# MarioPasc/MGA-YOLO

Measured on AMD Instinct MI355X. Metric: images/s (MaskCBAM fwd+bwd step at P3/P4/P5, YOLOv8n 640x640), higher is better.
Workload: dtype f32

## Files before the change

mga_yolo_amd/csrc/api_bwd.hip:

```cpp
#include "host.cuh"
#include "bwd.cuh"

static int backward_args(const mgacbam_bwd_level_t& L, BwdArgs& A, Sig& sig) {
  if (!L.x || !L.gy || !L.ctx || !L.scratch || !L.gx) return fail(MGACBAM_E_NULL, "backward: x / gy / ctx / scratch / gx is NULL");
  if (!L.gw1 || !L.gb1 || !L.gw2 || !L.gb2 || !L.gwsa || !L.gbeta) return fail(MGACBAM_E_NULL, "backward: NULL parameter-gradient pointer");
  if (L.gmask && !L.mask) return fail(MGACBAM_E_NULL, "backward: gmask requested but mask is NULL");
  if (int e = check_params(L.p)) return e;
  if (int e = check_shape(L.B, L.C, L.H, L.W, L.p.hidden, L.p.k)) return e;
  if (L.dtype < MGACBAM_F32 || L.dtype > MGACBAM_BF16) return fail(MGACBAM_E_DTYPE, "backward: dtype %d", L.dtype);
  const int VEC = vec_of(L.H, L.W, L.dtype);
  const size_t need = VEC * elem_size(L.dtype);
  if (!aligned_to(L.x, need) || !aligned_to(L.gy, need) || !aligned_to(L.gx, need) || !aligned_to(L.ctx, 16) ||
      !aligned_to(L.scratch, 16) || (L.gmask && !aligned_to(L.gmask, 16)))
    return fail(MGACBAM_E_ALIGN, "backward: x/gy/gx must be %zu-byte aligned, ctx/scratch 16-byte", need);
  A.x = L.x; A.mask = L.mask; A.gy = L.gy; A.gx = L.gx; A.gmask = L.gmask;
  A.gw1 = L.gw1; A.gb1 = L.gb1; A.gw2 = L.gw2; A.gb2 = L.gb2; A.gwsa = L.gwsa; A.gbeta = L.gbeta;
  A.c = ctx_ptrs(const_cast<void*>(L.ctx), L.B, L.C, L.H, L.W, L.p.hidden);
  A.p = make_params(L.p);
  A.g = make_geo(L.B, L.C, L.H, L.W, L.p);
  A.t = choose_tune(L.B, L.C, L.H, L.W, L.p.k, L.dtype);
  const ScratchLayout SL = scratch_layout(L.B, L.C, L.H, L.W, L.p.hidden, L.p.k, L.dtype);
  {
    mgacbam_ctx_layout_t CL;
    ctx_layout(L.B, L.C, L.H, L.W, L.p.hidden, &CL);
    if (int e = check_capacity("backward", "ctx", static_cast<size_t>(CL.total), L.ctx_bytes)) return e;
    if (int e = check_capacity("backward", "scratch", SL.total, L.scratch_bytes)) return e;
  }
  char* sp = static_cast<char*>(L.scratch);
  A.s.A_part = reinterpret_cast<float*>(sp + SL.A_part);
  A.s.gpre = reinterpret_cast<float*>(sp + SL.gpre); A.s.gplanes = reinterpret_cast<float*>(sp + SL.gplanes);
  A.s.gwsa_part = reinterpret_cast<float*>(sp + SL.gwsa_part);
  A.s.gz = reinterpret_cast<float*>(sp + SL.gz); A.s.gbq = reinterpret_cast<float*>(sp + SL.gbq);
  A.s.gh_avg = reinterpret_cast<float*>(sp + SL.gh_avg); A.s.gh_mx = reinterpret_cast<float*>(sp + SL.gh_mx);
  A.s.pgh = reinterpret_cast<float*>(sp + SL.pgh);
  A.nt = chan_tiles(A.t, A.g.H, A.g.W, VEC);
  A.nconv = A.g.B * conv_tiles(A.t, A.g.H, A.g.W);
  A.nwsa = A.g.B * wsa_tiles(A.t, A.g.H, A.g.W);
  A.nrole = A.nwsa;
  A.wsa_tail = 0;
  A.npg = params_blocks(A.g);
  A.ncg = 0;
  A.nflag = static_cast<int>(sync_flags(static_cast<size_t>(L.H) * L.W));
  A.bflag0 = L.B * A.nflag + 4 + L.B;
  A.cflag0 = A.bflag0 + L.B * A.nflag;
  A.mbflag0 = A.cflag0 + L.B * A.nflag; A.mcflag0 = A.mbflag0 + L.B * A.nflag;
  A.wflag0 = A.mcflag0 + L.B * A.nflag; A.sflag0 = A.wflag0 + L.B * A.nflag;
  A.merged = 0;
  A.vec = VEC;
  { const Knobs kn = knobs(); A.trace = kn.trace; A.spin_limit = kn.spin_limit; }
  const int proj = (L.flags & MGACBAM_BWD_HAVE_PROJ) && L.gmask != nullptr;
  A.g.proj_h = (proj && L.p.hidden <= MGACBAM_PROJ_MAX_HIDDEN) ? L.p.hidden : 0;
  sig = Sig{L.dtype, VEC, L.mask != nullptr, L.p.k, L.gmask != nullptr, proj};
  return 0;
}

static int backward_group(BwdArgs* lv, int n, const Sig& sig, int stages, hipStream_t st) {
  Group<BwdArgs> G;
  G.n = n;
  const int r2max = knobs().r2_cpt == 1 || knobs().r2_cpt == 2 || knobs().r2_cpt == 4 ? knobs().r2_cpt : 4;
  const int cpt = group_cpt(lv, n, r2max);
  for (int l = 0; l < n; ++l) {
    lv[l].t.pool_cpt = cpt;
    const int cpb = (kBlock / lv[l].t.pool_tx) * cpt;
    lv[l].ncg = (lv[l].g.C + cpb - 1) / cpb;
    G.lv[l] = lv[l];
  }
  auto fill = [&](auto blocks_of) { int tot = 0; for (int l = 0; l < n; ++l) { G.start[l] = tot; tot += blocks_of(lv[l]); } G.start[n] = tot; return tot; };

  bool fold = (stages & MGACBAM_BWD_FOLD) && (stages & MGACBAM_BWD_REDUCE1) && (stages & MGACBAM_BWD_CONVT) && knobs().bwd_fold;
  for (int l = 0; l < n && fold; ++l) {
    const int TP = lv[l].t.chan_tx * sig.vec;
    fold = TP >= kSyncPx && TP >= lv[l].g.W && 8 * (((lv[l].t.conv_th + lv[l].g.k) * lv[l].g.W + TP - 1) / TP + 1) <= 512 &&
           lv[l].nconv <= lv[l].g.B * lv[l].nflag;
  }
  const bool fuse_early = (stages & MGACBAM_BWD_FUSE) != 0;
  const bool tail_early = fuse_early && (stages & MGACBAM_BWD_APPLY) && (stages & MGACBAM_BWD_PARAMGRAD) && (stages & MGACBAM_BWD_WSA) && sig.k == 7 &&
                          knobs().wsa_tail;
  bool merge = fold && fuse_early && (stages & MGACBAM_BWD_REDUCE2) && (stages & MGACBAM_BWD_WSA) && sig.k == 7 && !tail_early && knobs().bwd_merge &&
               !knobs().wsa_fat;
  for (int l = 0; l < n && merge; ++l) merge = lv[l].nwsa <= lv[l].g.B * lv[l].nflag && lv[l].ncg <= lv[l].g.C && lv[l].nconv % lv[l].g.B == 0;
  if (merge) {
    R12Group R;
    R.g.n = n;
    size_t smem = 0;
    for (int l = 0; l < n; ++l) {
      lv[l].merged = 1; lv[l].bflag0 = lv[l].mbflag0; lv[l].cflag0 = lv[l].mcflag0; lv[l].nrole = lv[l].nwsa;
      R.g.lv[l] = lv[l];
      smem = std::max({smem, reduce1_smem(lv[l].g, sig.vec), convT_smem(lv[l].t, sig.k), wsa_smem(lv[l].t, sig.k),
                       (64 + static_cast<size_t>(std::max(kPghLds, kBlock / lv[l].t.pool_tx))) * sizeof(float)});
    }
    int tot = 0;
    for (int p = 0; p < 4; ++p) {
      for (int l = 0; l < n; ++l) {
        R.seg[p][l] = tot;
        tot += p == 0 ? xcd_grid(lv[l].g.B, lv[l].nt) : p == 1 ? pad8(lv[l].nconv) : p == 2 ? pad8(lv[l].nwsa) : sweep_blocks(lv[l], lv[l].t.pool_tx, cpt);
      }
      R.seg[p][n] = tot;
    }
    const int grid = tot;
#define CALL_R12B(CPTV) LAUNCH((k_bwd_r12<TT, VV, CPTV>), grid, smem, st, R)
#define CALL_R12(Tt, Vv) { using TT = Tt; constexpr int VV = Vv; DISPATCH_CPT(cpt, CALL_R12B); }
    DISPATCH_T_VEC(sig.dtype, sig.vec, CALL_R12);
#undef CALL_R12
#undef CALL_R12B
    if (int e = launch_status("k_bwd_r12")) return e;
    for (int l = 0; l < n; ++l) G.lv[l] = lv[l];
  }
  if (fold && !merge) {
    size_t smem = 0;
    for (int l = 0; l < n; ++l) smem = std::max({smem, reduce1_smem(lv[l].g, sig.vec), convT_smem(lv[l].t, sig.k)});
    const int grid = fill([&](const BwdArgs& a) { return xcd_grid(a.g.B, a.nt) + pad8(a.nconv); });
#define CALL_R1F(Tt, Vv) if (sig.k == 7) LAUNCH((k_bwd_reduce1_fold<Tt, Vv, 7>), grid, smem, st, G); else LAUNCH((k_bwd_reduce1_fold<Tt, Vv, 0>), grid, smem, st, G)
    DISPATCH_T_VEC(sig.dtype, sig.vec, CALL_R1F);
#undef CALL_R1F
    if (int e = launch_status("k_bwd_reduce1_fold")) return e;
  }
  if ((stages & MGACBAM_BWD_REDUCE1) && !fold) {
    size_t smem = 0;
    for (int l = 0; l < n; ++l) smem = std::max(smem, reduce1_smem(lv[l].g, sig.vec));
    const int grid = fill([&](const BwdArgs& a) { return xcd_grid(a.g.B, a.nt); });
#define CALL_R1(Tt, Vv) LAUNCH((k_bwd_reduce1<Tt, Vv>), grid, smem, st, G)
    DISPATCH_T_VEC(sig.dtype, sig.vec, CALL_R1);
#undef CALL_R1
    if (int e = launch_status("k_bwd_reduce1")) return e;
  }
  if ((stages & MGACBAM_BWD_CONVT) && !fold) {
    size_t smem = 0;
    for (int l = 0; l < n; ++l) smem = std::max(smem, convT_smem(lv[l].t, sig.k));
    const int grid = fill([&](const BwdArgs& a) { return a.nconv; });
    switch (sig.k) {
      case 3: LAUNCH(k_bwd_convT<3>, grid, smem, st, G); break;
      case 5: LAUNCH(k_bwd_convT<5>, grid, smem, st, G); break;
      case 7: LAUNCH(k_bwd_convT<7>, grid, smem, st, G); break;
      default: LAUNCH(k_bwd_convT<0>, grid, smem, st, G); break;
    }
    if (int e = launch_status("k_bwd_convT")) return e;
  }
  const bool fuse = (stages & MGACBAM_BWD_FUSE) != 0;
  const bool fuse_pg = fuse && (stages & MGACBAM_BWD_APPLY) && (stages & MGACBAM_BWD_PARAMGRAD);
  const bool wsa_tail = fuse_pg && (stages & MGACBAM_BWD_FOLD) && (stages & MGACBAM_BWD_WSA) && sig.k == 7 && knobs().wsa_tail;
  const bool fuse_wsa = fuse && (stages & MGACBAM_BWD_REDUCE2) && (stages & MGACBAM_BWD_WSA) && sig.k == 7 && !wsa_tail;
  if (wsa_tail) for (int l = 0; l < n; ++l) { lv[l].wsa_tail = 1; G.lv[l].wsa_tail = 1; }
  if ((stages & MGACBAM_BWD_REDUCE2) && !merge) {
    size_t smem = 0;
    for (int l = 0; l < n; ++l) {
      smem = std::max(smem, (64 + static_cast<size_t>(std::max(kPghLds, kBlock / lv[l].t.pool_tx))) * sizeof(float));
      if (fuse_wsa) smem = std::max(smem, wsa_smem(lv[l].t, sig.k));
    }
    if (fuse_wsa && knobs().wsa_fat) {
      int slots = 0;
#define RES_R22(CPTV) slots = resident_workgroups(k_bwd_reduce2<TT, VV, CPTV, true>, smem)
#define RES_R2(Tt, Vv) { using TT = Tt; constexpr int VV = Vv; DISPATCH_CPT(cpt, RES_R22); }
      DISPATCH_T_VEC(sig.dtype, sig.vec, RES_R2);
#undef RES_R2
#undef RES_R22
      long long streaming = 0, tiles = 0;
      for (int l = 0; l < n; ++l) {
        const int cpb = (kBlock / lv[l].t.pool_tx) * cpt;
        streaming += static_cast<long long>(lv[l].g.B) * ((lv[l].g.C + cpb - 1) / cpb);
        tiles += lv[l].nwsa;
      }
      const long long idle = slots - streaming;
      if (idle >= 32 && idle < tiles) {
        for (int l = 0; l < n; ++l) {
          lv[l].nrole = static_cast<int>(std::max(1ll, std::min<long long>(lv[l].nwsa, idle * lv[l].nwsa / tiles)));
          G.lv[l].nrole = lv[l].nrole;
        }
      }
    }
    const int grid = fill([&](const BwdArgs& a) { return (fuse_wsa ? pad8(a.nrole) : 0) + sweep_blocks(a, a.t.pool_tx, cpt); });
#define CALL_R22(CPTV) if (fuse_wsa) LAUNCH((k_bwd_reduce2<TT, VV, CPTV, true>), grid, smem, st, G); else LAUNCH((k_bwd_reduce2<TT, VV, CPTV, false>), grid, smem, st, G)
#define CALL_R2(Tt, Vv) { using TT = Tt; constexpr int VV = Vv; DISPATCH_CPT(cpt, CALL_R22); }
    DISPATCH_T_VEC(sig.dtype, sig.vec, CALL_R2);
#undef CALL_R2
#undef CALL_R22
    if (int e = launch_status("k_bwd_reduce2")) return e;
  }
  if ((stages & MGACBAM_BWD_WSA) && !fuse_wsa && !wsa_tail && !merge) {
    size_t smem = 0;
// ... 52 lines not shown
```

mga_yolo_amd/csrc/args.cuh:

```cuda
#pragma once
#include <stddef.h>
#include <stdint.h>

namespace mgacbam {

struct Geo {
  int B, C, H, W, HW;
  int hidden, k;
  int use_sigmoid;
  float thr, eps;
  int proj_h;
};
constexpr int kProjMax = 4;
#ifndef MGACBAM_GATE_R
#define MGACBAM_GATE_R 16
#endif
constexpr int kGateR = MGACBAM_GATE_R;
constexpr int kSyncPx = 16;

struct CtxPtrs {
  float* S; float* use; float* den;
  float* avg; float* mx; float* mavg;
  int* valid; int* amax;
  float* h_avg; float* h_mx; float* ca;
// ... 9 lines not shown
  int pool_cpt;
  int chan_tx;
  int chanf_tx;
  int conv_twq;
  int conv_th;
  int wsa_th;
  int apply_rows;
  int nt_stores;
  int gate_rows;
  int gate_tx;
  int gate_span;
};

struct FwdArgs {
  const void* x; const float* mask; void* y;
  CtxPtrs c; ParamPtrs p; Geo g; Tune t;
  int nflag;
  int fused;
  unsigned spin_limit;
  int fault;
  long long* trace;
};

struct ScratchPtrs {
  float* A_part;
  float* gpre;
  float* gplanes;
  float* gwsa_part;
  float* gz;
  float* gbq;
  float* gh_avg;
  float* gh_mx;
  float* pgh;
};

struct BwdArgs {
  const void* x; const float* mask; const void* gy; void* gx; float* gmask;
  float* gw1; float* gb1; float* gw2; float* gb2; float* gwsa; float* gbeta;
  CtxPtrs c; ParamPtrs p; ScratchPtrs s; Geo g; Tune t;
  int nt;
  int nconv;
  int nwsa;
  int nrole;
  int npg;
  int ncg;
  int nflag;
  int bflag0;
  int cflag0;
  int wflag0;
  int sflag0;
  int mbflag0, mcflag0;
  int merged;
  unsigned spin_limit;
  int vec;
  int wsa_tail;
  long long* trace;
};

static inline size_t align16(size_t v) { return (v + 15) & ~size_t(15); }

constexpr int kGroupMax = 4;
template <typename Args>
struct Group {
  int n;
  int start[kGroupMax + 1];
  Args lv[kGroupMax];
};

}
```

mga_yolo_amd/csrc/bwd.cuh:

```cuda
#pragma once
#include "args.cuh"
#include "common.cuh"
#include "tile.cuh"

#ifndef MGACBAM_BAPPLY_UNROLL
#define MGACBAM_BAPPLY_UNROLL 4
#endif
constexpr int kPghLds = 2048;

#ifndef MGACBAM_EARLY_H
#define MGACBAM_EARLY_H 8
#endif
#ifndef MGACBAM_BAPPLY_UN
#define MGACBAM_BAPPLY_UN 2
#endif

#ifdef MGACBAM_BWD_WAVES
#define BWD_OCC __attribute__((amdgpu_waves_per_eu(MGACBAM_BWD_WAVES, MGACBAM_BWD_WAVES)))
#else
#define BWD_OCC
#endif

namespace mgacbam {

// ... 38 lines not shown
    for (int e = 0; e < VEC; ++e) {
      const float p = xv[e] * gv[e] * live;
      accp[e] += cac * p;
      pa += p * sav[e];
      pq += p * (cac * sav[e] - 1.f);
    }
    pa = wave_group_sum(pa, TX);
    pq = wave_group_sum(pq, TX);
    if (tx == 0) { s_aq[c] = pa; s_aq[g.C + c] = pq; }
  }
#pragma unroll
  for (int e = 0; e < VEC; ++e) sm[tid * VEC + e] = accp[e];
  __syncthreads();
  float* part = A.s.A_part + (static_cast<size_t>(b) * ntile + tile) * 2 * g.C;
  if (FOLD && A.merged) { for (int c = tid; c < 2 * g.C; c += kBlock) st_agent(part + c, s_aq[c]); }
  else { for (int c = tid; c < 2 * g.C; c += kBlock) part[c] = s_aq[c]; }
  if (ty == 0 && active) {
    for (int r = 1; r < TY; ++r) {
      const int o = (r * TX + tx) * VEC;
#pragma unroll
      for (int e = 0; e < VEC; ++e) accp[e] += sm[o + e];
    }
    float gpre[VEC];
#pragma unroll
    for (int e = 0; e < VEC; ++e) gpre[e] = a * accp[e] * sav[e] * (1.f - sav[e]);
    float* gq = A.s.gpre + static_cast<size_t>(b) * g.HW + static_cast<size_t>(i) * VEC;
    if (FOLD) {
#pragma unroll
      for (int e = 0; e < VEC; ++e) st_agent(gq + e, gpre[e]);
    } else {
      store_vec<float, VEC>(gq, gpre);
    }
  }
  if (FOLD) handoff_publish(A.c.sync + A.bflag0 + static_cast<size_t>(b) * A.nflag + tile);
}

template <typename T, int VEC>
__global__ __launch_bounds__(kBlock) void k_bwd_reduce1(const Group<BwdArgs> G) {
  extern __shared__ __align__(16) float smem[];
  int local;
  const int l = find_level(G, blockIdx.x, local);
  bwd_reduce1_body<T, VEC>(G.lv[l], local, smem);
}

template <int K, bool COH>
__device__ __forceinline__ void bwd_convT_body(const BwdArgs& A, const int local, float* smem) {
  const Geo& g = A.g;
  const int k = K ? K : g.k;
  const ConvTile c = conv_tile(g, A.t, k, local, A.t.conv_th);
  const int tid = threadIdx.x;
  float* wts = smem;
  float* tg = smem + ((3 * k * k + 3) & ~3);
  for (int i = tid; i < 3 * k * k; i += kBlock) wts[i] = A.p.wsa[i];
  const float* gpre = A.s.gpre + static_cast<size_t>(c.b) * g.HW;
  bool bad = false;
  if (COH) {
    int* own = A.c.sync + A.cflag0 + local;
    const int gen = static_cast<int>(static_cast<unsigned>(ld_agent(own)) + 1u);
    const int TP = A.t.chan_tx * A.vec;
    const int ra = max(c.y0 - c.pad, 0), rb = min(c.y0 + c.TH - 1 + c.pad, g.H - 1);
    bad = handoff_wait(A.c.sync + A.bflag0 + static_cast<size_t>(c.b) * A.nflag, (ra * g.W) / TP, ((rb + 1) * g.W - 1) / TP, gen,
                       A.c.sync + static_cast<size_t>(g.B) * A.nflag, A.spin_limit);
    if (tid == 0 && !A.merged) __hip_atomic_fetch_add(own, 1, __ATOMIC_RELAXED, __HIP_MEMORY_SCOPE_AGENT);
  }
  stage_window<8>(tg, 1, c.PH, c.PW, c.y0 - c.pad, c.x0 - c.pad, g, [&](int, int off) { return COH ? ld_agent(gpre + off) : gpre[off]; });
  __syncthreads();
// ... 135 lines not shown
    }
    __syncthreads();
    for (int o = tid; o < nout; o += kBlock) {
      const int pi = o / KK, j = o - pi * KK;
      float sum = 0.f;
      for (int r = 0; r < c.TH; ++r) sum += accs[(pi * c.TH + r) * KK + j];
      if (COH && bad) sum = __builtin_nanf("");
      if (AGENT) st_agent(A.s.gwsa_part + static_cast<size_t>(o) * A.nwsa + local, sum);
      else A.s.gwsa_part[static_cast<size_t>(o) * A.nwsa + local] = sum;
    }
  } else {
    for (int o = tid; o < nout; o += kBlock) {
      const int p = o / (k * k), r = o - p * k * k;
      const int i = r / k, j = r - i * k;
      const float* pp = tp + p * plane_elems + i * c.PW + j;
      const float* gg = tg + c.pad * c.PW + c.pad;
      float sum = 0.f;
      for (int yy = 0; yy < c.TH; ++yy)
        for (int xx = 0; xx < c.TW; ++xx) sum += gg[yy * c.PW + xx] * pp[yy * c.PW + xx];
      if (AGENT) st_agent(A.s.gwsa_part + static_cast<size_t>(o) * A.nwsa + local, sum);
      else A.s.gwsa_part[static_cast<size_t>(o) * A.nwsa + local] = sum;
    }
  }
}

template <int K>
__global__ __launch_bounds__(kBlock) void k_bwd_wsa(const Group<BwdArgs> G) {
  extern __shared__ __align__(16) float smem[];
  int local;
  const int lvl = find_level(G, blockIdx.x, local);
  bwd_wsa_body<K>(G.lv[lvl], local, smem);
}

typedef unsigned int v4u32_t __attribute__((ext_vector_type(4)));
typedef float v4f32_t __attribute__((ext_vector_type(4)));
template <int VEC>
__device__ __forceinline__ void load_plane_agent(__amdgpu_buffer_rsrc_t rsrc, const int elem, float (&out)[VEC]) {
  if constexpr (VEC % 4 == 0) {
#pragma unroll
    for (int q = 0; q < VEC / 4; ++q) {
      const v4u32_t v = __builtin_amdgcn_raw_buffer_load_b128(rsrc, (elem + 4 * q) * 4, 0, 16);
      const v4f32_t f = __builtin_bit_cast(v4f32_t, v);
      out[4 * q] = f.x; out[4 * q + 1] = f.y; out[4 * q + 2] = f.z; out[4 * q + 3] = f.w;
    }
  } else {
#pragma unroll
    for (int e = 0; e < VEC; ++e) out[e] = __builtin_bit_cast(float, __builtin_amdgcn_raw_buffer_load_b32(rsrc, (elem + e) * 4, 0, 16));
  }
}

template <typename T, int VEC, int CPT, bool COH = false>
__device__ __forceinline__ void bwd_reduce2_body(const BwdArgs& A, const int bid, float* red) {
  const Geo& g = A.g;
  const int tid = threadIdx.x;
  const int TX = A.t.pool_tx, lt = ilog2(TX);
  const int tx = tid & (TX - 1), ty = tid >> lt, TY = kBlock >> lt;
  const int CPB = TY * CPT;
  const int ncg = (g.C + CPB - 1) / CPB;
  int b, cg;
  if (!xcd_sample_part(bid, g.B, ncg, b, cg)) return;
  const int c0 = cg * CPB + ty * CPT;
  const int nv = g.HW / VEC;
  const float invC = 1.f / static_cast<float>(g.C);

  const T* xr[CPT];
  int cj[CPT];
#pragma unroll
  for (int j = 0; j < CPT; ++j) {
    cj[j] = min(c0 + j, g.C - 1);
    xr[j] = static_cast<const T*>(A.x) + (static_cast<size_t>(b) * g.C + cj[j]) * g.HW;
  }
  const float* gp0 = A.s.gplanes + static_cast<size_t>(b) * 3 * g.HW;
  const float* gp1 = gp0 + g.HW;
  const int* cidx = A.c.cidx + static_cast<size_t>(b) * g.HW;
  float acc[CPT];
#pragma unroll
  for (int j = 0; j < CPT; ++j) acc[j] = 0.f;
  bool bad = false;
  __amdgpu_buffer_rsrc_t gprs = __builtin_amdgcn_make_buffer_rsrc(const_cast<float*>(gp0), 0, 2 * g.HW * 4, 0x00020000);
  if (COH) {
    int* own = A.c.sync + A.sflag0 + static_cast<size_t>(b) * g.C + cg;
    const int gen = static_cast<int>(static_cast<unsigned>(ld_agent(own)) + 1u);
    const int cps = A.nconv / g.B;
    bad = handoff_wait(A.c.sync + A.cflag0, b * cps, b * cps + cps - 1, gen, A.c.sync + static_cast<size_t>(g.B) * A.nflag, A.spin_limit);
    if (tid == 0) __hip_atomic_fetch_add(own, 1, __ATOMIC_RELAXED, __HIP_MEMORY_SCOPE_AGENT);
  }

  constexpr int PF = MGACBAM_POOL_PF;
  for (int i0 = tx; i0 < nv; i0 += TX * PF) {
    float g0[PF][VEC], g1[PF][VEC], xv[PF][CPT][VEC];
    int ci[PF][VEC];
    bool ok[PF];
#pragma unroll
    for (int p = 0; p < PF; ++p) {
      const int i = i0 + p * TX;
      ok[p] = i < nv;
      const size_t o = static_cast<size_t>(ok[p] ? i : nv - 1) * VEC;
      if (COH) {
        load_plane_agent<VEC>(gprs, static_cast<int>(o), g0[p]);
        load_plane_agent<VEC>(gprs, g.HW + static_cast<int>(o), g1[p]);
      } else {
        load_vec<float, VEC>(gp0 + o, g0[p]);
        load_vec<float, VEC>(gp1 + o, g1[p]);
      }
      load_ivec<VEC>(cidx + o, ci[p]);
#pragma unroll
      for (int j = 0; j < CPT; ++j) load_vec<T, VEC>(xr[j] + o, xv[p][j]);
    }
#pragma unroll
    for (int p = 0; p < PF; ++p) {
      if (!ok[p]) continue;
#pragma unroll
      for (int j = 0; j < CPT; ++j) {
#pragma unroll
        for (int e = 0; e < VEC; ++e) {
          const float wgt = g1[p][e] * invC + (ci[p][e] == cj[j] ? g0[p][e] : 0.f);
          acc[j] += xv[p][j][e] * wgt;
        }
// ... 17 lines not shown
    const float a = softplusf_(*A.p.beta);
#pragma unroll
    for (int j = 0; j < CPT; ++j) {
      const int c = c0 + j;
      if (c < g.C) {
        const size_t o = static_cast<size_t>(b) * g.C + c;
        const float As = sums[CPT + j], Qs = sums[2 * CPT + j];
        const float ca = A.c.ca[o];
        const float gca = a * As + sums[j];
        gzv[j] = (COH && bad) ? __builtin_nanf("") : gca * ca * (1.f - ca);
        A.s.gz[o] = gzv[j];
        A.s.gbq[o] = Qs;
      }
    }
  }
  const int h = g.hidden;
  float* s_pg = red + 64;
  const int hc = min(h, max(1, kPghLds / TY));
  for (int h0 = 0; h0 < h; h0 += hc) {
    const int hn = min(hc, h - h0);
    if (h0) __syncthreads();
    if (tx == 0) {
      for (int jh = 0; jh < hn; ++jh) {
        float p = 0.f;
#pragma unroll
        for (int j = 0; j < CPT; ++j) p += A.p.w2[static_cast<size_t>(cj[j]) * h + h0 + jh] * gzv[j];
        s_pg[ty * hc + jh] = p;
      }
    }
    __syncthreads();
    for (int jh = tid; jh < hn; jh += kBlock) {
      float p = 0.f;
      for (int r = 0; r < TY; ++r) p += s_pg[r * hc + jh];
      A.s.pgh[(static_cast<size_t>(b) * ncg + cg) * h + h0 + jh] = p;
    }
  }
}

template <typename T, int VEC, int CPT, bool ROLES>
__global__ __launch_bounds__(kBlock) BWD_OCC void k_bwd_reduce2(const Group<BwdArgs> G) {
  extern __shared__ __align__(16) float smem[];
  int local;
  const int l = find_level(G, blockIdx.x, local);
  const BwdArgs& A = G.lv[l];
  if (ROLES) {
    const int npad = (A.nrole + 7) & ~7;
    if (local < npad) {
      if (local < A.nrole) {
        TRACE_MARK(A.trace, blockIdx.x, 0);
        for (int t = local; t < A.nwsa; t += A.nrole) { bwd_wsa_body<7>(A, t, smem); __syncthreads(); }
#ifdef MGACBAM_TRACE
        asm volatile("s_waitcnt vmcnt(0)" ::: "memory");
        TRACE_MARK(A.trace, blockIdx.x, 5);
#endif
      }
      return;
    }
    local -= npad;
  }
  TRACE_MARK(A.trace, blockIdx.x, 0);
  bwd_reduce2_body<T, VEC, CPT>(A, local, smem);
#ifdef MGACBAM_TRACE
  asm volatile("s_waitcnt vmcnt(0)" ::: "memory");
  TRACE_MARK(A.trace, blockIdx.x, 10);
#endif
}

struct R12Group {
  Group<BwdArgs> g;
  int seg[4][kGroupMax + 1];
};
template <typename T, int VEC, int CPT>
__global__ __launch_bounds__(kBlock) BWD_OCC void k_bwd_r12(const R12Group R) {
  extern __shared__ __align__(16) float smem[];
  const int bid = blockIdx.x;
  int p = 0;
#pragma unroll
  for (int q = 1; q < 4; ++q)
    if (bid >= R.seg[q][0]) p = q;
  int l = 0;
#pragma unroll
  for (int i = 1; i < kGroupMax; ++i)
    if (i < R.g.n && bid >= R.seg[p][i]) l = i;
  const int local = bid - R.seg[p][l];
  const BwdArgs& A = R.g.lv[l];
#ifdef MGACBAM_TRACE
  TRACE_MARK(A.trace, blockIdx.x, 0);
  if (A.trace && threadIdx.x == 0) A.trace[static_cast<size_t>(blockIdx.x) * 16 + 14] = p + 1;
#endif
  if (p == 0) bwd_reduce1_body<T, VEC, true>(A, local, smem);
  else if (p == 1) { if (local < A.nconv) bwd_convT_body<7, true>(A, local, smem); }
  else if (p == 2) { if (local < A.nwsa) bwd_wsa_body<7, false, true>(A, local, smem); }
  else bwd_reduce2_body<T, VEC, CPT, true>(A, local, smem);
#ifdef MGACBAM_TRACE
  asm volatile("s_waitcnt vmcnt(0)" ::: "memory");
  __syncthreads();
  TRACE_MARK(A.trace, blockIdx.x, 10);
#endif
}

__device__ __forceinline__ void bwd_params_body(const BwdArgs& A, const int local, float* sm, float* red) {
  const Geo& g = A.g;
  const int C = g.C, h = g.hidden, B = g.B, kk3 = 3 * g.k * g.k;
  const int nb2 = (C + kBlock - 1) / kBlock, nb_wsa = (kk3 + 3) / 4;
  const int tid = threadIdx.x, wave = tid >> 6, lane = tid & 63;
  if (local < h) {
    const int j = local;
    float* s_ga = sm; float* s_gm = sm + B; float* s_hs = sm + 2 * B;
    float* s_part = sm + 3 * B;
#pragma unroll 2
    for (int b = wave; b < B; b += kBlock / kWave) {
      const float* gz = A.s.gz + static_cast<size_t>(b) * C;
      float d = 0.f;
#pragma unroll 4
      for (int c = lane; c < C; c += kWave) d += A.p.w2[static_cast<size_t>(c) * h + j] * gz[c];
      d = wave_group_sum(d, kWave);
      if (lane == 0) {
        const float ha = A.c.h_avg[b * h + j], hm = A.c.h_mx[b * h + j];
        const float ga = ha > 0.f ? d : 0.f, gm = hm > 0.f ? d : 0.f;
        s_ga[b] = ga; s_gm[b] = gm; s_hs[b] = ha + hm;
        A.s.gh_avg[b * h + j] = ga;
        A.s.gh_mx[b * h + j] = gm;
      }
    }
    __syncthreads();
    const int cp = (C >= kBlock) ? kBlock : C;
// ... 39 lines not shown
    A.gb2[c] = 2.f * acc;
    return;
  }
  if (local < h + nb2 + nb_wsa) {
    if (A.wsa_tail) return;
    const int o = (local - h - nb2) * 4 + wave;
    if (o >= kk3) return;
    const float* part = A.s.gwsa_part + static_cast<size_t>(o) * A.nwsa;
    float acc = 0.f;
#pragma unroll 4
    for (int t = lane; t < A.nwsa; t += kWave) acc += part[t];
    acc = wave_group_sum(acc, kWave);
    if (lane == 0) A.gwsa[o] = acc;
    return;
  }
  {
    float acc = 0.f;
#pragma unroll 8
    for (int o = tid; o < B * C; o += kBlock) acc += A.s.gbq[o];
    acc = block_sum(acc, tid, red);
    if (tid == 0) *A.gbeta = sigmoidf_(*A.p.beta) * acc;
  }
}

__global__ __launch_bounds__(kBlock) void k_bwd_params(const Group<BwdArgs> G) {
  extern __shared__ __align__(16) float sm[];
  __shared__ float red[8];
  int local;
  const int lvl = find_level(G, blockIdx.x, local);
  bwd_params_body(G.lv[lvl], local, sm, red);
}

template <typename T, int VEC, bool GMASK>
__device__ __forceinline__ void bwd_apply_body(const BwdArgs& A, const int bid, float* smem, float* red) {
  constexpr int UN = MGACBAM_BAPPLY_UN;
  const Geo& g = A.g;
  const int tid = threadIdx.x;
  const int TX = A.t.chan_tx, lt = ilog2(TX);
  const int tx = tid & (TX - 1), ty = tid >> lt, TY = kBlock >> lt;
  const int nv = g.HW / VEC;
  const int ntile = (nv + TX - 1) / TX;
  int b, tile;
  if (!xcd_sample_part(bid, g.B, ntile, b, tile)) return;
  const int i = tile * TX + tx;
  const bool active = i < nv;
  const int ii = active ? i : nv - 1;
  const size_t base = static_cast<size_t>(b) * g.C * g.HW + static_cast<size_t>(ii) * VEC;
  const T* xp = static_cast<const T*>(A.x) + base;
  const T* gp = static_cast<const T*>(A.gy) + base;
  T* op = static_cast<T*>(A.gx) + base;
  const float a = softplusf_(*A.p.beta);
  const float N = static_cast<float>(g.HW);
  const bool has_mask = A.mask != nullptr;
  const size_t po = static_cast<size_t>(b) * g.HW + static_cast<size_t>(ii) * VEC;

  const int gid = blockIdx.x;
  TRACE_HWID(A.trace, gid);
  TRACE_MARK(A.trace, gid, 0);
  float sav[VEC], g0[VEC], g1[VEC], sv[VEC], wA[VEC];
  int ci[VEC];
  load_vec<float, VEC>(A.c.sa + po, sav);
  load_vec<float, VEC>(A.s.gplanes + static_cast<size_t>(b) * 3 * g.HW + static_cast<size_t>(ii) * VEC, g0);
  load_vec<float, VEC>(A.s.gplanes + (static_cast<size_t>(b) * 3 + 1) * g.HW + static_cast<size_t>(ii) * VEC, g1);
  load_vec<float, VEC>(A.c.planes + (static_cast<size_t>(b) * 3 + 2) * g.HW + static_cast<size_t>(ii) * VEC, sv);
  load_ivec<VEC>(A.c.cidx + po, ci);
  const float use = A.c.use[b], den = A.c.den[b];
  const float invC = 1.f / static_cast<float>(g.C);
#pragma unroll
  for (int e = 0; e < VEC; ++e) {
    g1[e] *= invC;
    sav[e] *= a;
    wA[e] = has_mask ? (use * sv[e] / den + (1.f - use) / N) : 1.f / N;
  }
  const int* amax = A.c.amax + static_cast<size_t>(b) * g.C;
  float accp[VEC];
#pragma unroll
  for (int e = 0; e < VEC; ++e) accp[e] = 0.f;

  const bool need_x = GMASK && g.proj_h == 0;
  float g0v[UN][VEC], x0v[UN][VEC];
#pragma unroll
  for (int u = 0; u < UN; ++u) {
    const size_t co = static_cast<size_t>(min(ty + u * TY, g.C - 1)) * g.HW;
    load_vec<T, VEC>(gp + co, g0v[u]);
    if (GMASK) { if (need_x) load_vec<T, VEC>(xp + co, x0v[u]); }
  }

  float4* s_q = reinterpret_cast<float4*>(smem);
  int* s_am = reinterpret_cast<int*>(smem + 4 * g.C);
  float* s_gh = smem + 5 * g.C;
  float* sm = s_gh + 2 * g.hidden;
  const int h = g.hidden;
  const float live = (has_mask && A.c.S[b] >= g.eps) ? 1.f : 0.f;
  float kpart = 0.f;
  constexpr int kEarlyH = MGACBAM_EARLY_H;
  const bool early = g.C <= kBlock && h <= kEarlyH;
  float rw1[kEarlyH], rca = 0.f, rmavg = 0.f;
  int rvalid = 0, ramax = 0;
  if (early) {
    const int c = min(tid, g.C - 1);
    const size_t o = static_cast<size_t>(b) * g.C + c;
    rca = A.c.ca[o]; rmavg = A.c.mavg[o]; rvalid = A.c.valid[o]; ramax = amax[c];
#pragma unroll
    for (int j = 0; j < kEarlyH; ++j) rw1[j] = A.p.w1[static_cast<size_t>(min(j, h - 1)) * g.C + c];
  }
  {
    const float* pg = A.s.pgh + static_cast<size_t>(b) * A.ncg * h;
    const int hh = h < kBlock ? h : kBlock;
    const int G_ = kBlock / hh;
    const int j0 = tid % hh, k0 = tid / hh;
    for (int jb = 0; jb < h; jb += hh) {
      const int j = jb + j0;
      float p = 0.f;
      if (k0 < G_ && j < h)
        for (int cg = k0; cg < A.ncg; cg += G_) p += pg[cg * h + j];
      sm[tid] = p;
      __syncthreads();
      if (k0 == 0 && j < h) {
        for (int q = 1; q < G_; ++q) p += sm[q * hh + j0];
        s_gh[j] = A.c.h_avg[static_cast<size_t>(b) * h + j] > 0.f ? p : 0.f;
        s_gh[h + j] = A.c.h_mx[static_cast<size_t>(b) * h + j] > 0.f ? p : 0.f;
      }
      __syncthreads();
    }
  }
  TRACE_MARK(A.trace, gid, 1);
  if (early) {
    if (tid < g.C) {
      float ga = 0.f, gm = 0.f;
#pragma unroll
      for (int j = 0; j < kEarlyH; ++j)
        if (j < h) { ga += rw1[j] * s_gh[j]; gm += rw1[j] * s_gh[h + j]; }
      float4 q;
      q.x = rca;
      q.y = ga;
      q.z = rvalid ? gm : 0.f;
      q.w = rvalid ? 0.f : gm / N;
      s_q[tid] = q;
      s_am[tid] = rvalid ? ramax : -1;
      kpart += ga * rmavg * live;
    }
  } else {
    for (int c = tid; c < g.C; c += kBlock) {
      float ga = 0.f, gm = 0.f;
      for (int j = 0; j < h; ++j) { const float wv = A.p.w1[static_cast<size_t>(j) * g.C + c]; ga += wv * s_gh[j]; gm += wv * s_gh[h + j]; }
      const size_t o = static_cast<size_t>(b) * g.C + c;
      const int valid = A.c.valid[o];
      float4 q;
      q.x = A.c.ca[o];
      q.y = ga;
      q.z = valid ? gm : 0.f;
      q.w = valid ? 0.f : gm / N;
      s_q[c] = q;
      s_am[c] = valid ? amax[c] : -1;
      kpart += ga * A.c.mavg[o] * live;
    }
  }

  kpart = block_sum(kpart, tid, red);
  if (tid == 0) red[7] = kpart;
  __syncthreads();
  const float kb = red[7];
  TRACE_MARK(A.trace, gid, 2);

  auto emit = [&](const float (&gv)[VEC], const float (&xv)[VEC], int c) {
    float ov[VEC];
    const float4 q = s_q[c];
    const int am = s_am[c] - ii * VEC;
#pragma unroll
    for (int e = 0; e < VEC; ++e) {
      float r = gv[e] * ((1.f - a) + sav[e] * q.x);
      r += q.x * ((ci[e] == c ? g0[e] : 0.f) + g1[e]);
      r += q.y * wA[e] + q.w;
      r += (am == e) ? q.z : 0.f;
      ov[e] = r;
      if (GMASK) { if (need_x) accp[e] += q.y * xv[e]; }
    }
    if (active) store_vec_stream<T, VEC>(op + static_cast<size_t>(c) * g.HW, ov, A.t.nt_stores);
  };
#pragma unroll
  for (int u = 0; u < UN; ++u) {
    const int c = ty + u * TY;
    if (c < g.C) emit(g0v[u], x0v[u], c);
  }
#pragma unroll MGACBAM_BAPPLY_UNROLL
  for (int c = ty + UN * TY; c < g.C; c += TY) {
    float gv[VEC], xv[VEC];
    load_vec<T, VEC>(gp + static_cast<size_t>(c) * g.HW, gv);
    if (GMASK) { if (need_x) load_vec<T, VEC>(xp + static_cast<size_t>(c) * g.HW, xv); }
    emit(gv, xv, c);
  }
  TRACE_MARK(A.trace, gid, 3);
  if (GMASK) {
    if (need_x) {
#pragma unroll
// ... 71 lines not shown

template <typename T, int VEC, bool GMASK, bool ROLES>
__global__ __launch_bounds__(kBlock) void k_bwd_apply(const Group<BwdArgs> G) {
  extern __shared__ __align__(16) float smem[];
  __shared__ float red[8];
  int local;
  const int l = find_level(G, blockIdx.x, local);
  const BwdArgs& A = G.lv[l];
  if (ROLES) {
    const int npad = (A.npg + 7) & ~7;
    if (local < npad) {
      if (local < A.npg) {
        TRACE_MARK(A.trace, blockIdx.x, 0);
        bwd_params_body(A, local, smem, red);
#ifdef MGACBAM_TRACE
        asm volatile("s_waitcnt vmcnt(0)" ::: "memory");
        __syncthreads();
        TRACE_MARK(A.trace, blockIdx.x, 9);
#endif
      }
      return;
    }
    local -= npad;
    if (A.wsa_tail) {
      const int tiles = ((A.g.B + 7) / 8) * 8 * A.nt;
      if (local >= tiles) {
        const int nsum = (3 * A.g.k * A.g.k + 3) / 4;
        if (local - tiles < A.nwsa) bwd_wsa_tail(A, local - tiles, smem);
        else if (local - tiles - A.nwsa < nsum) bwd_wsa_sum(A, local - tiles - A.nwsa, nsum);
        return;
      }
    }
  }
  bwd_apply_body<T, VEC, GMASK>(A, local, smem, red);
}

}
```

mga_yolo_amd/csrc/host.cuh:

```cuda
#pragma once
#include "../../include/mgacbam.h"

#include <hip/hip_runtime.h>
#include <stdarg.h>
#include <stdio.h>
#include <stdlib.h>
#include <string.h>

#include <algorithm>
#include <atomic>
#include <map>
#include <mutex>
#include <utility>

#include "args.cuh"
#include "common.cuh"

using namespace mgacbam;

inline thread_local char g_err[512] = "";
static int fail(int code, const char* fmt, ...) {
  va_list ap;
  va_start(ap, fmt);
  vsnprintf(g_err, sizeof(g_err), fmt, ap);
// ... 187 lines not shown
  t.conv_th = th;
  int wth = 3500 / (4 * (tw + k - 1)) - (k - 1);
  if (wth > H) wth = H;
  if (wth > 64) wth = 64;
  if (wth < 1) wth = 1;
  t.wsa_th = wth;
  int v;
  if (is_pow2_in(v = kn.pool_tx, 1, 256)) t.pool_tx = v;
  if ((v = kn.pool_cpt) == 1 || v == 2 || v == 4) t.pool_cpt = v;
  if (is_pow2_in(v = kn.chan_tx, 1, 64)) t.chan_tx = v;
  t.chanf_tx = t.chan_tx;
  if (is_pow2_in(v = kn.chanf_tx, 1, 64)) t.chanf_tx = v;
  int rows = (t.chan_tx * VEC - 1) / W + 2;
  if (rows > H) rows = H;
  t.apply_rows = rows + k - 1;
  t.nt_stores = kn.nt ? 1 : 0;
  gate_geometry(C, H, W, k, VEC, t);
  return t;
}

static int conv_tiles(const Tune& t, int H, int W) {
  const int TW = t.conv_twq * 4;
  return ((W + TW - 1) / TW) * ((H + t.conv_th - 1) / t.conv_th);
}
static int wsa_tiles(const Tune& t, int H, int W) {
  const int TW = t.conv_twq * 4;
  return ((W + TW - 1) / TW) * ((H + t.wsa_th - 1) / t.wsa_th);
}
static int chan_tiles(const Tune& t, int H, int W, int vec) {
  const int nv = H * W / vec;
  return (nv + t.chan_tx - 1) / t.chan_tx;
}

struct ScratchLayout { size_t A_part, gpre, gplanes, gwsa_part, gz, gbq, gh_avg, gh_mx, pgh, total; };
static ScratchLayout scratch_layout(int B, int C, int H, int W, int hidden, int k, int dtype) {
  const Tune t = choose_tune(B, C, H, W, k, dtype);
  const size_t HW = static_cast<size_t>(H) * W, BC = static_cast<size_t>(B) * C;
  const size_t nt = chan_tiles(t, H, W, vec_of(H, W, dtype)), nconv = static_cast<size_t>(B) * wsa_tiles(t, H, W);
  ScratchLayout L;
  size_t o = 0;
  auto take = [&](size_t n_elems) { size_t at = o; o = align16(o + n_elems * 4); return at; };
  L.A_part = take(2 * BC * nt);
  L.gpre = take(B * HW); L.gplanes = take(static_cast<size_t>(B) * 3 * HW);
  L.gwsa_part = take(nconv * 3 * k * k);
  L.gz = take(BC); L.gbq = take(BC);
  L.gh_avg = take(static_cast<size_t>(B) * hidden); L.gh_mx = take(static_cast<size_t>(B) * hidden);
  const size_t ty = kBlock / t.pool_tx;
  L.pgh = take(static_cast<size_t>(B) * ((C + ty - 1) / ty) * hidden);
  L.total = o;
  return L;
}

static int check_capacity(const char* what, const char* buf, size_t want, size_t got) {
  if (got < want)
    return fail(MGACBAM_E_SIZE, "%s: %s holds %zu bytes, this shape needs %zu under the current knobs (query the size again after "
                "mgacbam_reload_env(); a size cached across a knob change or taken for another shape is stale)", what, buf, got, want);
  return 0;
}

static size_t elem_size(int dtype) { return dtype == MGACBAM_F32 ? 4 : 2; }
static bool aligned_to(const void* p, size_t a) { return (reinterpret_cast<uintptr_t>(p) % a) == 0; }

#define LAUNCH(kernel, grid, smem, stream, args) launch(kernel, static_cast<unsigned>(grid), smem, stream, args)

#define DISPATCH_T_VEC(dtype, VECV, CALL)                                                         \
  do {                                                                                            \
    if ((dtype) == MGACBAM_F32) { if ((VECV) == 4) { CALL(float, 4); } else { CALL(float, 1); } }  \
    else if ((dtype) == MGACBAM_F16) { if ((VECV) == 8) { CALL(__half, 8); } else if ((VECV) == 4) { CALL(__half, 4); } else { CALL(__half, 1); } } \
    else { if ((VECV) == 8) { CALL(bf16_t, 8); } else if ((VECV) == 4) { CALL(bf16_t, 4); } else { CALL(bf16_t, 1); } }          \
  } while (0)

#define DISPATCH_CPT(CPTV, CALL2)                                              \
  do { if ((CPTV) == 4) { CALL2(4); } else if ((CPTV) == 2) { CALL2(2); } else { CALL2(1); } } while (0)

static Geo make_geo(int B, int C, int H, int W, const mgacbam_params_t& p) {
  Geo g;
  g.B = B; g.C = C; g.H = H; g.W = W; g.HW = H * W; g.hidden = p.hidden; g.k = p.k;
  g.use_sigmoid = p.use_sigmoid_mask; g.thr = p.tiny_thr; g.eps = p.eps;
  g.proj_h = 0;
  return g;
}
// ... 85 lines not shown
```

Measured before the change: 160,900.

## Compute per-sample channel-attention terms once in last reduce2 block

Moves the per-sample reduction of hidden-layer gradients, the w1 matvec and the kpart block sum out of every apply block into the last-arriving reduce2 block of each sample, chosen with an atomic arrival counter. The result is written to a per-sample record in scratch, and apply blocks just copy it into shared memory. This removes work that every apply tile used to repeat, at the cost of a serialized tail in one block per sample, extra atomics and a new scratch region. The merge condition is loosened so it no longer requires ncg <= C.

```diff
diff --git a/mga_yolo_amd/csrc/api_bwd.hip b/mga_yolo_amd/csrc/api_bwd.hip
--- a/mga_yolo_amd/csrc/api_bwd.hip
+++ b/mga_yolo_amd/csrc/api_bwd.hip
@@ -33,6 +33,7 @@
   A.s.gz = reinterpret_cast<float*>(sp + SL.gz); A.s.gbq = reinterpret_cast<float*>(sp + SL.gbq);
   A.s.gh_avg = reinterpret_cast<float*>(sp + SL.gh_avg); A.s.gh_mx = reinterpret_cast<float*>(sp + SL.gh_mx);
   A.s.pgh = reinterpret_cast<float*>(sp + SL.pgh);
+  A.s.rec = reinterpret_cast<float*>(sp + SL.rec);
   A.nt = chan_tiles(A.t, A.g.H, A.g.W, VEC);
   A.nconv = A.g.B * conv_tiles(A.t, A.g.H, A.g.W);
   A.nwsa = A.g.B * wsa_tiles(A.t, A.g.H, A.g.W);
@@ -44,7 +45,8 @@
   A.bflag0 = L.B * A.nflag + 4 + L.B;
   A.cflag0 = A.bflag0 + L.B * A.nflag;
   A.mbflag0 = A.cflag0 + L.B * A.nflag; A.mcflag0 = A.mbflag0 + L.B * A.nflag;
-  A.wflag0 = A.mcflag0 + L.B * A.nflag; A.sflag0 = A.wflag0 + L.B * A.nflag;
+  A.wflag0 = A.mcflag0 + L.B * A.nflag;
+  A.arr0 = A.wflag0 + L.B * A.nflag; A.sgen0 = A.arr0 + L.B;
   A.merged = 0;
   A.vec = VEC;
   { const Knobs kn = knobs(); A.trace = kn.trace; A.spin_limit = kn.spin_limit; }
@@ -52,6 +54,10 @@
   A.g.proj_h = (proj && L.p.hidden <= MGACBAM_PROJ_MAX_HIDDEN) ? L.p.hidden : 0;
   sig = Sig{L.dtype, VEC, L.mask != nullptr, L.p.k, L.gmask != nullptr, proj};
   return 0;
+}
+
+static size_t reduce2_smem(const BwdArgs& a) {
+  return std::max(64 + static_cast<size_t>(std::max(kPghLds, kBlock / a.t.pool_tx)), 8 + static_cast<size_t>(kBlock) + 2 * a.g.hidden) * sizeof(float);
 }
 
 static int backward_group(BwdArgs* lv, int n, const Sig& sig, int stages, hipStream_t st) {
@@ -78,7 +84,7 @@
                           knobs().wsa_tail;
   bool merge = fold && fuse_early && (stages & MGACBAM_BWD_REDUCE2) && (stages & MGACBAM_BWD_WSA) && sig.k == 7 && !tail_early && knobs().bwd_merge &&
                !knobs().wsa_fat;
-  for (int l = 0; l < n && merge; ++l) merge = lv[l].nwsa <= lv[l].g.B * lv[l].nflag && lv[l].ncg <= lv[l].g.C && lv[l].nconv % lv[l].g.B == 0;
+  for (int l = 0; l < n && merge; ++l) merge = lv[l].nwsa <= lv[l].g.B * lv[l].nflag && lv[l].g.C >= 2 && lv[l].nconv % lv[l].g.B == 0;
   if (merge) {
     R12Group R;
     R.g.n = n;
@@ -86,8 +92,7 @@
     for (int l = 0; l < n; ++l) {
       lv[l].merged = 1; lv[l].bflag0 = lv[l].mbflag0; lv[l].cflag0 = lv[l].mcflag0; lv[l].nrole = lv[l].nwsa;
       R.g.lv[l] = lv[l];
-      smem = std::max({smem, reduce1_smem(lv[l].g, sig.vec), convT_smem(lv[l].t, sig.k), wsa_smem(lv[l].t, sig.k),
-                       (64 + static_cast<size_t>(std::max(kPghLds, kBlock / lv[l].t.pool_tx))) * sizeof(float)});
+      smem = std::max({smem, reduce1_smem(lv[l].g, sig.vec), convT_smem(lv[l].t, sig.k), wsa_smem(lv[l].t, sig.k), reduce2_smem(lv[l])});
     }
     int tot = 0;
     for (int p = 0; p < 4; ++p) {
@@ -144,7 +149,7 @@
   if ((stages & MGACBAM_BWD_REDUCE2) && !merge) {
     size_t smem = 0;
     for (int l = 0; l < n; ++l) {
-      smem = std::max(smem, (64 + static_cast<size_t>(std::max(kPghLds, kBlock / lv[l].t.pool_tx))) * sizeof(float));
+      smem = std::max(smem, reduce2_smem(lv[l]));
       if (fuse_wsa) smem = std::max(smem, wsa_smem(lv[l].t, sig.k));
     }
     if (fuse_wsa && knobs().wsa_fat) {
diff --git a/mga_yolo_amd/csrc/args.cuh b/mga_yolo_amd/csrc/args.cuh
--- a/mga_yolo_amd/csrc/args.cuh
+++ b/mga_yolo_amd/csrc/args.cuh
@@ -65,7 +65,9 @@
   float* gh_avg;
   float* gh_mx;
   float* pgh;
+  float* rec;
 };
+__host__ __device__ inline int rec_floats(int C, int hidden) { return (4 + 5 * C + 2 * hidden + 3) & ~3; }
 
 struct BwdArgs {
   const void* x; const float* mask; const void* gy; void* gx; float* gmask;
@@ -81,7 +83,8 @@
   int bflag0;
   int cflag0;
   int wflag0;
-  int sflag0;
+  int arr0;
+  int sgen0;
   int mbflag0, mcflag0;
   int merged;
   unsigned spin_limit;
diff --git a/mga_yolo_amd/csrc/bwd.cuh b/mga_yolo_amd/csrc/bwd.cuh
--- a/mga_yolo_amd/csrc/bwd.cuh
+++ b/mga_yolo_amd/csrc/bwd.cuh
@@ -94,6 +94,7 @@
       store_vec<float, VEC>(gq, gpre);
     }
   }
+  if (tile == 0 && tid == 0 && !A.merged) st_agent(A.c.sync + A.arr0 + b, 0);
   if (FOLD) handoff_publish(A.c.sync + A.bflag0 + static_cast<size_t>(b) * A.nflag + tile);
 }
 
@@ -295,6 +296,61 @@
   bwd_wsa_body<K>(G.lv[lvl], local, smem);
 }
 
+__device__ __forceinline__ void bwd_sample_terms(const BwdArgs& A, const int b, float* smem) {
+  const Geo& g = A.g;
+  const int tid = threadIdx.x, h = g.hidden;
+  float* red = smem;
+  float* sm = smem + 8;
+  float* s_gh = sm + kBlock;
+  float* rec = A.s.rec + static_cast<size_t>(b) * rec_floats(g.C, h);
+  float4* r_q = reinterpret_cast<float4*>(rec + 4);
+  int* r_am = reinterpret_cast<int*>(rec + 4 + 4 * g.C);
+  float* r_gh = rec + 4 + 5 * g.C;
+  const float N = static_cast<float>(g.HW);
+  const bool has_mask = A.mask != nullptr;
+  const float live = (has_mask && A.c.S[b] >= g.eps) ? 1.f : 0.f;
+  {
+    const float* pg = A.s.pgh + static_cast<size_t>(b) * A.ncg * h;
+    const int hh = h < kBlock ? h : kBlock;
+    const int G_ = kBlock / hh;
+    const int j0 = tid % hh, k0 = tid / hh;
+    for (int jb = 0; jb < h; jb += hh) {
+      const int j = jb + j0;
+      float p = 0.f;
+      if (k0 < G_ && j < h)
+        for (int cg = k0; cg < A.ncg; cg += G_) p += ld_agent(pg + cg * h + j);
+      sm[tid] = p;
+      __syncthreads();
+      if (k0 == 0 && j < h) {
+        for (int q = 1; q < G_; ++q) p += sm[q * hh + j0];
+        const float ga = A.c.h_avg[static_cast<size_t>(b) * h + j] > 0.f ? p : 0.f;
+        const float gm = A.c.h_mx[static_cast<size_t>(b) * h + j] > 0.f ? p : 0.f;
+        s_gh[j] = ga; s_gh[h + j] = gm;
+        r_gh[j] = ga; r_gh[h + j] = gm;
+      }
+      __syncthreads();
+    }
+  }
+  const int* amax = A.c.amax + static_cast<size_t>(b) * g.C;
+  float kpart = 0.f;
+  for (int c = tid; c < g.C; c += kBlock) {
+    float ga = 0.f, gm = 0.f;
+    for (int j = 0; j < h; ++j) { const float wv = A.p.w1[static_cast<size_t>(j) * g.C + c]; ga += wv * s_gh[j]; gm += wv * s_gh[h + j]; }
+    const size_t o = static_cast<size_t>(b) * g.C + c;
+    const int valid = A.c.valid[o];
+    float4 q;
+    q.x = A.c.ca[o];
+    q.y = ga;
+    q.z = valid ? gm : 0.f;
+    q.w = valid ? 0.f : gm / N;
+    r_q[c] = q;
+    r_am[c] = valid ? amax[c] : -1;
+    kpart += ga * A.c.mavg[o] * live;
+  }
+  kpart = block_sum(kpart, tid, red);
+  if (tid == 0) rec[0] = kpart;
+}
+
 typedef unsigned int v4u32_t __attribute__((ext_vector_type(4)));
 typedef float v4f32_t __attribute__((ext_vector_type(4)));
 template <int VEC>
@@ -313,7 +369,7 @@
 }
 
 template <typename T, int VEC, int CPT, bool COH = false>
-__device__ __forceinline__ void bwd_reduce2_body(const BwdArgs& A, const int bid, float* red) {
+__device__ __forceinline__ int bwd_reduce2_body(const BwdArgs& A, const int bid, float* red) {
   const Geo& g = A.g;
   const int tid = threadIdx.x;
   const int TX = A.t.pool_tx, lt = ilog2(TX);
@@ -321,7 +377,7 @@
   const int CPB = TY * CPT;
   const int ncg = (g.C + CPB - 1) / CPB;
   int b, cg;
-  if (!xcd_sample_part(bid, g.B, ncg, b, cg)) return;
+  if (!xcd_sample_part(bid, g.B, ncg, b, cg)) return -1;
   const int c0 = cg * CPB + ty * CPT;
   const int nv = g.HW / VEC;
   const float invC = 1.f / static_cast<float>(g.C);
@@ -342,11 +398,9 @@
   bool bad = false;
   __amdgpu_buffer_rsrc_t gprs = __builtin_amdgcn_make_buffer_rsrc(const_cast<float*>(gp0), 0, 2 * g.HW * 4, 0x00020000);
   if (COH) {
-    int* own = A.c.sync + A.sflag0 + static_cast<size_t>(b) * g.C + cg;
-    const int gen = static_cast<int>(static_cast<unsigned>(ld_agent(own)) + 1u);
+    const int gen = static_cast<int>(static_cast<unsigned>(ld_agent(A.c.sync + A.sgen0 + b)) + 1u);
     const int cps = A.nconv / g.B;
     bad = handoff_wait(A.c.sync + A.cflag0, b * cps, b * cps + cps - 1, gen, A.c.sync + static_cast<size_t>(g.B) * A.nflag, A.spin_limit);
-    if (tid == 0) __hip_atomic_fetch_add(own, 1, __ATOMIC_RELAXED, __HIP_MEMORY_SCOPE_AGENT);
   }
 
   constexpr int PF = MGACBAM_POOL_PF;
@@ -430,9 +484,22 @@
     for (int jh = tid; jh < hn; jh += kBlock) {
       float p = 0.f;
       for (int r = 0; r < TY; ++r) p += s_pg[r * hc + jh];
-      A.s.pgh[(static_cast<size_t>(b) * ncg + cg) * h + h0 + jh] = p;
-    }
-  }
+      st_agent(A.s.pgh + (static_cast<size_t>(b) * ncg + cg) * h + h0 + jh, p);
+    }
+  }
+  int* cnt = A.c.sync + A.arr0 + b;
+  asm volatile("s_waitcnt vmcnt(0)" ::: "memory");
+  __syncthreads();
+  int last = 0;
+  if (tid == 0) last = __hip_atomic_fetch_add(cnt, 1, __ATOMIC_RELAXED, __HIP_MEMORY_SCOPE_AGENT) == ncg - 1;
+  if (__syncthreads_or(last)) {
+    if (tid == 0) {
+      st_agent(cnt, 0);
+      if (COH) __hip_atomic_fetch_add(A.c.sync + A.sgen0 + b, 1, __ATOMIC_RELAXED, __HIP_MEMORY_SCOPE_AGENT);
+    }
+    return b;
+  }
+  return -1;
 }
 
 template <typename T, int VEC, int CPT, bool ROLES>
@@ -457,7 +524,8 @@
     local -= npad;
   }
   TRACE_MARK(A.trace, blockIdx.x, 0);
-  bwd_reduce2_body<T, VEC, CPT>(A, local, smem);
+  const int last = bwd_reduce2_body<T, VEC, CPT>(A, local, smem);
+  if (last >= 0) bwd_sample_terms(A, last, smem);
 #ifdef MGACBAM_TRACE
   asm volatile("s_waitcnt vmcnt(0)" ::: "memory");
   TRACE_MARK(A.trace, blockIdx.x, 10);
@@ -489,7 +557,10 @@
   if (p == 0) bwd_reduce1_body<T, VEC, true>(A, local, smem);
   else if (p == 1) { if (local < A.nconv) bwd_convT_body<7, true>(A, local, smem); }
   else if (p == 2) { if (local < A.nwsa) bwd_wsa_body<7, false, true>(A, local, smem); }
-  else bwd_reduce2_body<T, VEC, CPT, true>(A, local, smem);
+  else {
+    const int last = bwd_reduce2_body<T, VEC, CPT, true>(A, local, smem);
+    if (last >= 0) bwd_sample_terms(A, last, smem);
+  }
 #ifdef MGACBAM_TRACE
   asm volatile("s_waitcnt vmcnt(0)" ::: "memory");
   __syncthreads();
@@ -595,7 +666,7 @@
 }
 
 template <typename T, int VEC, bool GMASK>
-__device__ __forceinline__ void bwd_apply_body(const BwdArgs& A, const int bid, float* smem, float* red) {
+__device__ __forceinline__ void bwd_apply_body(const BwdArgs& A, const int bid, float* smem) {
   constexpr int UN = MGACBAM_BAPPLY_UN;
   const Geo& g = A.g;
   const int tid = threadIdx.x;
@@ -635,7 +706,6 @@
     sav[e] *= a;
     wA[e] = has_mask ? (use * sv[e] / den + (1.f - use) / N) : 1.f / N;
   }
-  const int* amax = A.c.amax + static_cast<size_t>(b) * g.C;
   float accp[VEC];
 #pragma unroll
   for (int e = 0; e < VEC; ++e) accp[e] = 0.f;
@@ -649,81 +719,20 @@
     if (GMASK) { if (need_x) load_vec<T, VEC>(xp + co, x0v[u]); }
   }
 
+  const int h = g.hidden;
+  const float* rec = A.s.rec + static_cast<size_t>(b) * rec_floats(g.C, h);
+  const float kb = rec[0];
+  {
+    const float4* src = reinterpret_cast<const float4*>(rec + 4);
+    float4* dst = reinterpret_cast<float4*>(smem);
+    const int n4 = (5 * g.C + 2 * h + 3) / 4;
+    for (int i = tid; i < n4; i += kBlock) dst[i] = src[i];
+  }
   float4* s_q = reinterpret_cast<float4*>(smem);
   int* s_am = reinterpret_cast<int*>(smem + 4 * g.C);
   float* s_gh = smem + 5 * g.C;
   float* sm = s_gh + 2 * g.hidden;
-  const int h = g.hidden;
-  const float live = (has_mask && A.c.S[b] >= g.eps) ? 1.f : 0.f;
-  float kpart = 0.f;
-  constexpr int kEarlyH = MGACBAM_EARLY_H;
-  const bool early = g.C <= kBlock && h <= kEarlyH;
-  float rw1[kEarlyH], rca = 0.f, rmavg = 0.f;
-  int rvalid = 0, ramax = 0;
-  if (early) {
-    const int c = min(tid, g.C - 1);
-    const size_t o = static_cast<size_t>(b) * g.C + c;
-    rca = A.c.ca[o]; rmavg = A.c.mavg[o]; rvalid = A.c.valid[o]; ramax = amax[c];
-#pragma unroll
-    for (int j = 0; j < kEarlyH; ++j) rw1[j] = A.p.w1[static_cast<size_t>(min(j, h - 1)) * g.C + c];
-  }
-  {
-    const float* pg = A.s.pgh + static_cast<size_t>(b) * A.ncg * h;
-    const int hh = h < kBlock ? h : kBlock;
-    const int G_ = kBlock / hh;
-    const int j0 = tid % hh, k0 = tid / hh;
-    for (int jb = 0; jb < h; jb += hh) {
-      const int j = jb + j0;
-      float p = 0.f;
-      if (k0 < G_ && j < h)
-        for (int cg = k0; cg < A.ncg; cg += G_) p += pg[cg * h + j];
-      sm[tid] = p;
-      __syncthreads();
-      if (k0 == 0 && j < h) {
-        for (int q = 1; q < G_; ++q) p += sm[q * hh + j0];
-        s_gh[j] = A.c.h_avg[static_cast<size_t>(b) * h + j] > 0.f ? p : 0.f;
-        s_gh[h + j] = A.c.h_mx[static_cast<size_t>(b) * h + j] > 0.f ? p : 0.f;
-      }
-      __syncthreads();
-    }
-  }
-  TRACE_MARK(A.trace, gid, 1);
-  if (early) {
-    if (tid < g.C) {
-      float ga = 0.f, gm = 0.f;
-#pragma unroll
-      for (int j = 0; j < kEarlyH; ++j)
-        if (j < h) { ga += rw1[j] * s_gh[j]; gm += rw1[j] * s_gh[h + j]; }
-      float4 q;
-      q.x = rca;
-      q.y = ga;
-      q.z = rvalid ? gm : 0.f;
-      q.w = rvalid ? 0.f : gm / N;
-      s_q[tid] = q;
-      s_am[tid] = rvalid ? ramax : -1;
-      kpart += ga * rmavg * live;
-    }
-  } else {
-    for (int c = tid; c < g.C; c += kBlock) {
-      float ga = 0.f, gm = 0.f;
-      for (int j = 0; j < h; ++j) { const float wv = A.p.w1[static_cast<size_t>(j) * g.C + c]; ga += wv * s_gh[j]; gm += wv * s_gh[h + j]; }
-      const size_t o = static_cast<size_t>(b) * g.C + c;
-      const int valid = A.c.valid[o];
-      float4 q;
-      q.x = A.c.ca[o];
-      q.y = ga;
-      q.z = valid ? gm : 0.f;
-      q.w = valid ? 0.f : gm / N;
-      s_q[c] = q;
-      s_am[c] = valid ? amax[c] : -1;
-      kpart += ga * A.c.mavg[o] * live;
-    }
-  }
-
-  kpart = block_sum(kpart, tid, red);
-  if (tid == 0) red[7] = kpart;
-  __syncthreads();
-  const float kb = red[7];
+  __syncthreads();
   TRACE_MARK(A.trace, gid, 2);
 
   auto emit = [&](const float (&gv)[VEC], const float (&xv)[VEC], int c) {
@@ -861,7 +870,7 @@
       }
     }
   }
-  bwd_apply_body<T, VEC, GMASK>(A, local, smem, red);
-}
-
-}
+  bwd_apply_body<T, VEC, GMASK>(A, local, smem);
+}
+
+}
diff --git a/mga_yolo_amd/csrc/host.cuh b/mga_yolo_amd/csrc/host.cuh
--- a/mga_yolo_amd/csrc/host.cuh
+++ b/mga_yolo_amd/csrc/host.cuh
@@ -243,7 +243,7 @@
   return (nv + t.chan_tx - 1) / t.chan_tx;
 }
 
-struct ScratchLayout { size_t A_part, gpre, gplanes, gwsa_part, gz, gbq, gh_avg, gh_mx, pgh, total; };
+struct ScratchLayout { size_t A_part, gpre, gplanes, gwsa_part, gz, gbq, gh_avg, gh_mx, pgh, rec, total; };
 static ScratchLayout scratch_layout(int B, int C, int H, int W, int hidden, int k, int dtype) {
   const Tune t = choose_tune(B, C, H, W, k, dtype);
   const size_t HW = static_cast<size_t>(H) * W, BC = static_cast<size_t>(B) * C;
@@ -258,6 +258,7 @@
   L.gh_avg = take(static_cast<size_t>(B) * hidden); L.gh_mx = take(static_cast<size_t>(B) * hidden);
   const size_t ty = kBlock / t.pool_tx;
   L.pgh = take(static_cast<size_t>(B) * ((C + ty - 1) / ty) * hidden);
+  L.rec = take(static_cast<size_t>(B) * rec_floats(C, hidden));
   L.total = o;
   return L;
 }
```

Result: no change. 160,100 (median of 6 runs) (-0.5%).
